# jenkinsm13/julia-spira

Measured on AMD Instinct MI355X. Metric: Msamples/sec at 1920x1080 spp=64 depth=8; fraction of HBM roofline, higher is better.
Workload: dtype f64

## Files before the change

### include/spira_hip.h

```cpp
#ifndef SPIRA_HIP_H
#define SPIRA_HIP_H

#include <stdint.h>

#ifdef __cplusplus
extern "C" {
#endif

#define SPIRA_ABI_VERSION 3

#define SPIRA_OK            0
#define SPIRA_E_INVALID    -1
#define SPIRA_E_NO_DEVICE  -2
#define SPIRA_E_HIP        -3
#define SPIRA_E_LIMIT      -4
#define SPIRA_E_UNSUPPORTED -5

#define SPIRA_SEM_MASK          0x0000000Fu
#define SPIRA_SEM_A             0x00000000u
#define SPIRA_SEM_CPU           0x00000001u
#define SPIRA_SEM_METAL         0x00000002u
#define SPIRA_SEM_HYBRID        0x00000003u
#define SPIRA_KERNEL_MASK       0x000000F0u
#define SPIRA_KERNEL_DEFAULT    0x00000000u
// ... 233 lines not shown
int spira_render_adaptive_f64(const double *spheres5, const double *materials8, const double *triangles10,
                              const double camera12[12], const spira_params *params, const spira_adaptive *adaptive,
                              double *out_hdr, double *out_img, uint32_t *out_spp, double *out_q);
int spira_render_adaptive_scene_f32(const spira_scene *scene, const float camera12[12], const spira_params *params, const spira_adaptive *adaptive,
                                    float *out_hdr, float *out_img, uint32_t *out_spp, float *out_q);
int spira_render_adaptive_scene_f64(const spira_scene *scene, const double camera12[12], const spira_params *params, const spira_adaptive *adaptive,
                                    double *out_hdr, double *out_img, uint32_t *out_spp, double *out_q);
int spira_render_adaptive_scene_device_f32(const spira_scene *scene, const float camera12[12], const spira_params *params, const spira_adaptive *adaptive,
                                           float *d_out_hdr, float *d_out_img, uint32_t *d_out_spp, float *d_out_q, void *stream);
int spira_render_adaptive_scene_device_f64(const spira_scene *scene, const double camera12[12], const spira_params *params, const spira_adaptive *adaptive,
                                           double *d_out_hdr, double *d_out_img, uint32_t *d_out_spp, double *d_out_q, void *stream);
int spira_adaptive_converged_f32(const float sum3[3], float q, uint32_t n, double tolerance, double floor);
int spira_adaptive_converged_f64(const double sum3[3], double q, uint32_t n, double tolerance, double floor);

int spira_sky_pixel_f64(const double camera12[12], uint32_t width, uint32_t height, uint32_t i, uint32_t j, const double *spheres5, uint32_t n_spheres);

int spira_render_features_f32(const float *spheres5, const float *materials8, const float *triangles10,
                              const float camera12[12], const spira_params *params,
                              float *out_albedo, float *out_normal, float *out_depth);
int spira_render_features_f64(const double *spheres5, const double *materials8, const double *triangles10,
                              const double camera12[12], const spira_params *params,
                              double *out_albedo, double *out_normal, double *out_depth);
int spira_render_features_scene_f32(const spira_scene *scene, const float camera12[12], const spira_params *params,
                                    float *out_albedo, float *out_normal, float *out_depth);
int spira_render_features_scene_f64(const spira_scene *scene, const double camera12[12], const spira_params *params,
                                    double *out_albedo, double *out_normal, double *out_depth);
int spira_render_features_scene_device_f32(const spira_scene *scene, const float camera12[12], const spira_params *params,
                                           float *d_out_albedo, float *d_out_normal, float *d_out_depth, void *stream);
int spira_render_features_scene_device_f64(const spira_scene *scene, const double camera12[12], const spira_params *params,
                                           double *d_out_albedo, double *d_out_normal, double *d_out_depth, void *stream);
// ... 30 lines not shown
```

### julia-spira_amd/csrc/spira_device.h

```cpp
#pragma once
#include <hip/hip_runtime.h>
#include <stdint.h>
#include <type_traits>
#include "spira_fastdiv.h"
#include "spira_sky.h"

namespace spira {

__device__ __forceinline__ float sqrt_rn(float x) { return __builtin_sqrtf(x); }
__device__ __forceinline__ double sqrt_rn(double x) { return __builtin_sqrt(x); }

constexpr int kBlock = 256;
#ifndef SPIRA_WAVES_F32
#define SPIRA_WAVES_F32 5
#endif
#ifndef SPIRA_WAVES_F64
#define SPIRA_WAVES_F64 4
#endif
#define SPIRA_WAVES_PER_SIMD(T) (sizeof(T) == 8 ? SPIRA_WAVES_F64 : SPIRA_WAVES_F32)
constexpr uint32_t kMaxTries = 64;

template <class T> struct Vec { T x, y, z; };

template <class T> __device__ __forceinline__ Vec<T> mk(T x, T y, T z) { Vec<T> r; r.x = x; r.y = y; r.z = z; return r; }
// ... 723 lines not shown
    if (TRI && sc.n_triangles) {
        Pack4<T> v0n = sc.tri[0], e1n = sc.tri[1], e2n = sc.tri[2];
#pragma unroll 2
        for (uint32_t i = 0; i < sc.n_triangles; ++i) {
            const Pack4<T> v0 = v0n, e1 = e1n, e2 = e2n;
            const uint32_t nx = i + 1 < sc.n_triangles ? i + 1 : i;
            v0n = sc.tri[3 * nx]; e1n = sc.tri[3 * nx + 1]; e2n = sc.tri[3 * nx + 2];
            T t;
            if (triangle_test<T>(v0, e1, e2, o, d, t_min, closest, t, pol)) {
                closest = t; prim = (int)(sc.n_spheres + i);
            }
        }
    }
}

template <class T>
__device__ __forceinline__ bool mesh_box_hit(const SceneLds<T> &sc, Vec<T> o, Vec<T> d, T closest) {
    const Vec<T> inv = mk<T>(rcp_fast(d.x), rcp_fast(d.y), rcp_fast(d.z));
    return box_entry<T>(sc.bvh_root[0], sc.bvh_root[1], o, inv, closest) >= (T)0;
}

template <class T>
__device__ __forceinline__ void closest_hit_local(const SceneLds<T> &sc, Vec<T> o, Vec<T> d, T t_min, T &closest, int &prim) {
    ExactDiv exact;
    closest_hit_local<T>(sc, o, d, t_min, closest, prim, exact);
}
template <class T, bool BVH, class P, bool TRI = true>
__device__ __forceinline__ int closest_hit(const SceneLds<T> &sc, Vec<T> o, Vec<T> d, T t_min, T &t_hit, uint32_t &slot, P &pol) {
    T closest; int prim;
    closest_hit_local<T, P, TRI>(sc, o, d, t_min, closest, prim, pol);
// ... 236 lines not shown
    uint32_t pl = q - slot * rc.tile_pixels;
    uint32_t lr = fastdiv(pl, rc.fd_width);
    uint32_t lx = pl - lr * rc.width;
    j = ref_row_j(rc, lr);
    i = lx + 1;
    pixel = (j - 1) * rc.width + lx;
    sample = rc.sample0 + pass * rc.slots + slot;
}

template <class T> struct RayQueue { Pack4<T> *A; Pack4<T> *B; Pack2<T> *C; };

struct Stats {
    unsigned long long segments, rays_enqueued, radiance_rmw, radiance_store, redone_waves, rays_parked;
    unsigned long long mesh_wave_trips, mesh_lane_trips;
    unsigned long long sky_pixels;
};

template <class T> struct BounceArgs {
    SceneGlobal<T> scene;
    RenderConst<T> rc;
    RayQueue<T> qin, qout;
    Pack3<T> *L;
    const uint32_t *cnt_in;
    uint32_t *cnt_out;
    uint32_t *blk_stats;
    uint32_t cap;
    Stats *stats;
    uint32_t bounce;
    uint32_t pass;
    uint32_t n_first;
// ... 257 lines not shown
    Pack4<T> *mesh_list;
    uint32_t mesh_min_batch;
    uint32_t refill_free;
    uint32_t mesh_mode;
    uint32_t *mesh_count;
    uint32_t resume_k, resume_nw;
    uint32_t *redo;
    uint32_t redo_only;
    Stats *stats;
    Pack4<T> *accum;
    FastDiv fd_keff;
    uint32_t k_eff;
    uint32_t accum_first;
    uint32_t l_private;
    uint32_t sky_runs;
};

#ifndef SPIRA_RESOLVE_RUN
#define SPIRA_RESOLVE_RUN 4
#endif
__device__ __forceinline__ uint32_t owned_pixel(uint32_t w, uint32_t nw, uint32_t l) {
    constexpr uint32_t kRun = SPIRA_RESOLVE_RUN;
    static_assert(64 % kRun == 0, "a run length divides the wave");
    return ((l / kRun) * nw + w) * kRun + l % kRun;
}

template <class T>
__device__ __forceinline__ void resolve_pixel(Pack4<T> *accum, const Pack3<T> *L, uint32_t tile_pixels, uint32_t k_eff, bool first_pass, uint32_t p) {
    Pack4<T> acc;
    if (first_pass) { acc.x = 0; acc.y = 0; acc.z = 0; acc.w = 0; } else acc = accum[p];
// ... 104 lines not shown
    const bool mixed = mesh_mode != 0u || rc.max_depth <= 128u;
    const uint32_t dense_pct = mixed ? a.dense_pct : 0u;
    const bool defer = mesh_mode != 0u || (BVH && mixed && a.mesh_list != nullptr);
    Pack4<T> *mlist = a.mesh_list + 3 * (size_t)region;
    uint32_t n_rmw = 0, n_store = 0, n_seg = 0, n_enq = 0, n_park = 0;
    uint32_t n_wtrips = 0, n_ltrips = 0;
    uint32_t n_in = 0;
    const bool own = !BVH && !EXT && !TRI && sizeof(T) == 8 && a.accum != nullptr;
    const uint32_t n_own = own ? 64u * a.k_eff : 0u;
    const uint32_t n_sub_first = own ? (n_own + SUB - 1) / SUB : (a.n_first + SUB - 1) / SUB;
    const bool priv = kCarry && own && a.l_private != 0;
    const uint32_t l_base = priv ? wid * n_own : 0u;
    constexpr bool kOwnT = !BVH && !EXT && !TRI && sizeof(T) == 8;
    uint32_t sky_mask = 0;
    uint32_t *sky_word = reinterpret_cast<uint32_t *>(cam_lds + 12) + wave;
    static_assert(12 * sizeof(T) + WPB * sizeof(uint32_t) <= 128 || !kOwnT, "a word per wave behind the camera");
    if constexpr (kOwnT) {
        if (own && a.sky_runs) {
            constexpr uint32_t kRun = SPIRA_RESOLVE_RUN, kRuns = 64 / kRun, kRowSlots = 64 / kRun;
            static_assert(kRun == 4 && 2 * 64 * sizeof(Pack3<T>) <= SUB * sizeof(Pack4<T>), "the run mask below is written for runs of 4; a row of terms fits the work list");
            {
                const uint32_t px = owned_pixel(wid, NW, lane);
                bool sky = false;
                if (px < rc.tile_pixels) {
                    uint32_t pi, pj, pixel, sample;
                    path_of<T>(rc, px, a.pass, pi, pj, pixel, sample);
                    sky = sky_pixel(cam_lds, rc.width, rc.height, pi, pj, a.scene.spheres5, a.scene.n_spheres);
                }
                unsigned long long b = __ballot(sky);
                b &= b >> 1; b &= b >> 2;
                for (uint32_t g = 0; g < kRuns; ++g) sky_mask |= (uint32_t)((b >> (kRun * g)) & 1ull) << g;
            }
            Pack3<T> *s_sky = reinterpret_cast<Pack3<T> *>(s_rnd);
            for (uint32_t m = sky_mask; m; m &= m - 1u) {
                const uint32_t g = (uint32_t)__builtin_ctz(m);
                const uint32_t px = owned_pixel(wid, NW, g * kRun + lane % kRun);
                uint32_t pi, pj, pixel, sample0;
                path_of<T>(rc, px, a.pass, pi, pj, pixel, sample0);
                Pack3<T> acc;
                acc.x = 0; acc.y = 0; acc.z = 0;
                if (!a.accum_first && lane < kRun) { const Pack4<T> a0 = a.accum[px]; acc.x = a0.x; acc.y = a0.y; acc.z = a0.z; }
                for (uint32_t s0 = 0; s0 < a.k_eff; s0 += kRowSlots) {
                    const uint32_t slot = s0 + lane / kRun;
                    if (slot < a.k_eff) {
                        Vec<T> o_, d_;
                        camera_ray_lds<T>(rc, cam_lds, pix_div, pi, pj, pixel, sample0 + slot, o_, d_, pol);
                        const Vec<T> c = sky_term_x<T, EXT>(d_, mk<T>(1, 1, 1), nullptr);
                        Pack3<T> l; l.x = c.x; l.y = c.y; l.z = c.z;
                        s_sky[lane] = l;
                        ++n_seg; ++n_store;
                    }
                    wave_lds_sync();
                    if (lane < kRun) {
                        const uint32_t n = a.k_eff - s0 < kRowSlots ? a.k_eff - s0 : kRowSlots;
                        for (uint32_t k = 0; k < n; ++k) { const Pack3<T> l = s_sky[k * kRun + lane]; acc.x = acc.x + l.x; acc.y = acc.y + l.y; acc.z = acc.z + l.z; }
                    }
                    wave_lds_sync();
                }
                if (lane < kRun) a.L[priv ? l_base + g * a.k_eff * kRun + lane : px] = acc;
            }
        }
        if (own) { if (lane == 0) *sky_word = sky_mask; wave_lds_sync(); }
    }

    auto park = [&](uint32_t slot_i, const Vec<T> o_, const Vec<T> d_, const Vec<T> beta_, T closest_, uint32_t q_, int prim_, uint32_t stage_hit) {
        Pack4<T> A, B, C;
        A.x = o_.x; A.y = o_.y; A.z = o_.z; A.w = d_.x;
        B.x = d_.y; B.y = d_.z; B.z = beta_.x; B.w = beta_.y;
        C.x = beta_.z; C.y = closest_; C.z = Bits<T>::from_u32(q_); C.w = Bits<T>::from_u32((uint32_t)(prim_ + 1) | (stage_hit << kStageShift));
        mlist[3 * (size_t)slot_i] = A; mlist[3 * (size_t)slot_i + 1] = B; mlist[3 * (size_t)slot_i + 2] = C;
    };
    uint32_t mfill = 0;
    constexpr int kMaxSeg = 16;
    uint32_t pfx[kMaxSeg + 1];
    bool segmented = false;
    {
        uint32_t cnt = 0;
// ... 26 lines not shown
            Vec<T> o[R], beta[R];
            Pending<T> pend[R];
            ExtState<T> ex[R];
            uint32_t q[R], ent[R], stg[R], ref[R];
            uint32_t ka[R], kb[R];
            bool valid[R];
#pragma unroll
            for (int r = 0; r < R; ++r) {
                const uint32_t idx = sub * SUB + r * 64 + lane;
                valid[r] = false; stg[r] = round; ref[r] = 0; q[r] = 0; ka[r] = 0; kb[r] = 0;
                pend[r].kind = kDead; pend[r].rough = 0; pend[r].v = mk<T>(0, 0, 0);
                o[r] = mk<T>(0, 0, 0); beta[r] = mk<T>(1, 1, 1);
                bool parked = false; T park_t = 0; int park_prim = -1;
                uint32_t qf = idx;
                bool in = idx < limit;
                if (own && first) {
                    const uint32_t t = idx / SPIRA_RESOLVE_RUN, run = fastdiv(t, a.fd_keff);
                    const uint32_t px = owned_pixel(wid, NW, run * SPIRA_RESOLVE_RUN + idx % SPIRA_RESOLVE_RUN);
                    qf = (t - run * a.k_eff) * rc.tile_pixels + px;
                    in = in && px < rc.tile_pixels;
                    if constexpr (kOwnT) in = in && !((*sky_word >> run) & 1u);
                }
                const uint32_t ql = priv ? l_base + idx : qf;
                if (in) {
                    if (first) {
                        uint32_t pixel, sample, pi, pj;
                        Vec<T> d;
                        q[r] = ql;
                        path_of<T>(rc, qf, a.pass, pi, pj, pixel, sample);
                        if (kCarry) { ka[r] = mix32(rc.sA + pixel) ^ (sample << 8); kb[r] = mix32(rc.sB ^ pixel) + (sample << 8); }
                        camera_ray_lds<T>(rc, cam_lds, pix_div, pi, pj, pixel, sample, o[r], d, pol);
                        if (EXT) { ex[r].flags = rc.flags; if (rc.flags & kExtSpectral) beta[r] = ext_wavelength<T>(sc, rc.sA, rc.sB, pixel, sample, ex[r]); }
                        T t; uint32_t slot = 0;
                        int prim;
                        if (defer) {
                            if (kCam && a.cam_consts) closest_hit_local<T, Pol, TRI, true>(sc, o[r], d, (T)0.001, t, prim, pol, cam_sph);
                            else closest_hit_local<T, Pol, TRI>(sc, o[r], d, (T)0.001, t, prim, pol);
                            parked = mesh_box_hit<T>(sc, o[r], d, t);
                        } else if (kCam && !BVH && a.cam_consts) { closest_hit_local<T, Pol, TRI, true>(sc, o[r], d, (T)0.001, t, prim, pol, cam_sph); }
                        else prim = closest_hit<T, BVH, Pol, TRI>(sc, o[r], d, (T)0.001, t, slot, pol);
                        ++n_seg;
                        if (parked) { park_t = t; park_prim = prim; pend[r].v = d; }
                        else if (prim < 0) {
                            const Vec<T> c = sky_term_x<T, EXT>(d, beta[r], &ex[r]);
                            Pack3<T> l; l.x = c.x; l.y = c.y; l.z = c.z;
                            a.L[ql] = l;
                            ++n_store;
                        } else {
                            valid[r] = true;
                            o[r] = o[r] + d * t;
                            ref[r] = (BVH && prim >= (int)ref_base) ? ref_base + slot : (uint32_t)prim;
                            pend[r].v = d;
                        }
                    } else {
// ... 364 lines not shown
        const uint32_t px = owned_pixel(wid, NW, lane);
        bool summed = false;
        if constexpr (kOwnT) sky_mask = (uint32_t)__builtin_amdgcn_readfirstlane((int)*sky_word);
        if constexpr (kOwnT) summed = ((sky_mask >> (lane / SPIRA_RESOLVE_RUN)) & 1u) != 0;
        if (summed) {
            const Pack3<T> l = a.L[priv ? l_base + (lane / SPIRA_RESOLVE_RUN) * a.k_eff * SPIRA_RESOLVE_RUN + lane % SPIRA_RESOLVE_RUN : px];
            Pack4<T> acc;
            if (a.accum_first) acc.w = 0; else acc = a.accum[px];
            acc.x = l.x; acc.y = l.y; acc.z = l.z;
            a.accum[px] = acc;
        } else if (px < rc.tile_pixels) {
            if (priv) resolve_pixel_run<T>(a.accum, a.L + l_base + (lane / SPIRA_RESOLVE_RUN) * a.k_eff * SPIRA_RESOLVE_RUN + lane % SPIRA_RESOLVE_RUN, a.k_eff, a.accum_first != 0, px);
            else resolve_pixel<T>(a.accum, a.L, rc.tile_pixels, a.k_eff, a.accum_first != 0, px);
        }
        const uint32_t seg = __shfl(n_seg, 0), rmw = __shfl(n_rmw, 0), sto = __shfl(n_store, 0);
        if (lane < 4) {
            unsigned long long *f = lane == 0 ? &a.stats->segments : (lane == 1 ? &a.stats->rays_enqueued : (lane == 2 ? &a.stats->radiance_rmw : &a.stats->radiance_store));
            atomicAdd(f, (unsigned long long)(lane == 0 ? seg : (lane == 1 ? n_enq : (lane == 2 ? rmw : sto))));
        }
        if constexpr (kOwnT) if (lane == 4 && sky_mask) atomicAdd(&a.stats->sky_pixels, (unsigned long long)(SPIRA_RESOLVE_RUN * __popc(sky_mask)));
    }
    MESH_STAT(if (lane == 0) { unsigned long long *g = g_mesh_dbg + (mesh_mode == 2u ? 16 : 0);
                               atomicAdd(&g[0], __builtin_readcyclecounter() - dbg_t0); atomicAdd(&g[1], dbg_sess); atomicAdd(&g[2], (unsigned long long)dbg_ns);
                               atomicAdd(&g[3], (unsigned long long)dbg_ws); atomicAdd(&g[4], (unsigned long long)dbg_ls); atomicAdd(&g[5], (unsigned long long)dbg_rf);
                               atomicAdd(&g[6], (unsigned long long)dbg_rays); atomicAdd(&g[7], (unsigned long long)dbg_rounds); atomicAdd(&g[9], dbg_walk); atomicAdd(&g[10], 1ull); atomicAdd(&g[11], (unsigned long long)dbg_ws1); atomicAdd(&g[12], (unsigned long long)dbg_ls1);
                               atomicAdd(&g[8], (unsigned long long)dbg_h[0]); atomicAdd(&g[13], (unsigned long long)dbg_h[1]); atomicAdd(&g[14], (unsigned long long)dbg_h[2]); atomicAdd(&g[15], (unsigned long long)dbg_h[3]); })
    if (lane == 0) {
        if (mesh_mode == 2u) {
            const uint32_t row = 4 * wid * kseg;
            a.blk_stats[row] += n_seg; a.blk_stats[row + 1] += n_rmw; a.blk_stats[row + 2] += n_store; a.blk_stats[row + 3] += n_enq;
        } else {
            a.blk_stats[4 * wid] = n_seg;
            a.blk_stats[4 * wid + 1] = n_rmw;
            a.blk_stats[4 * wid + 2] = n_store;
            a.blk_stats[4 * wid + 3] = n_enq;
// ... 824 lines not shown
```

### julia-spira_amd/csrc/spira_hip.hip

```cpp
#include <hip/hip_runtime.h>
#include <sys/mman.h>
#include <rccl/rccl.h>
#include <dlfcn.h>

#include <algorithm>
#include <atomic>
#include <chrono>
#include <cmath>
#include <cstdio>
#include <cstdlib>
#include <cstring>
#include <condition_variable>
#include <mutex>
#include <new>
#include <string>
#include <thread>
#include <type_traits>
#include <vector>

#include "../../include/spira_hip.h"
#include "../../include/spira_spd.h"
#include "spira_device.h"
#include "spira_bvh.h"
#include "spira_validate.h"
// ... 132 lines not shown
    struct LbvhSmall *h_lbvh = nullptr;
    std::vector<void *> lbvh_retired;
    SceneStore scene;
    spira::Stats *h_stats = nullptr;
    void *h_stage = nullptr; size_t h_stage_cap = 0;
    std::vector<hipEvent_t> stage_ev;
    hipEvent_t ev_start = nullptr, ev_stop = nullptr;
    hipEvent_t ev_done = nullptr;
    bool have_done = false;
    std::vector<hipEvent_t> ev_pool;
    size_t ev_used = 0;
    std::vector<hipEvent_t> ev_mid;
    std::vector<size_t> ev_mid_end;
    size_t ev_mid_used = 0;
    spira_counters last{};
    uint64_t last_sky_pixels = 0;
    bool last_valid = false, last_pending = false;
    hipStream_t last_stream = nullptr;
    std::recursive_mutex mu;
};

constexpr int kMaxDevices = 16;
inline Ctx g_ctx[kMaxDevices];

}
using namespace spira_host;
namespace spira_tu {
int lbvh_topology(Ctx &c, hipStream_t st, uint32_t n, const LbvhWs &w, LbvhTopo &out);
}

// ... 478 lines not shown

spira::Knobs read_knobs() {
    spira::Knobs k;
    k.batch_rays = env_u32("SPIRA_BATCH_RAYS", k.batch_rays);
    k.R = env_u32("SPIRA_R", k.R);
    k.blocks_per_cu = env_u32("SPIRA_BLOCKS_PER_CU", 0);
    k.defer_mesh = env_u32("SPIRA_DEFER_MESH", 1); k.mesh_two_pass = env_u32("SPIRA_MESH_TWO_PASS", 1);
    k.fused_resolve = env_u32("SPIRA_FUSED_RESOLVE", 1); k.private_l = env_u32("SPIRA_PRIVATE_L", 1);
    k.spec_div = env_u32("SPIRA_SPEC_DIV", 1);
    k.dense_pct = std::min<uint32_t>(env_u32("SPIRA_DENSE_PCT", 70), 100);
    k.mesh_min_batch = std::max<uint32_t>(1, env_u32("SPIRA_MESH_MIN_BATCH", 128));
    k.mesh_refill = std::min<uint32_t>(64, std::max<uint32_t>(1, env_u32("SPIRA_MESH_REFILL", 16)));
    k.mesh_fat_waves_per_cu = env_u32("SPIRA_MESH_FAT_WAVES_PER_CU", 16);
    k.cam_consts = env_u32("SPIRA_CAM_CONSTS", 1);
    k.sky_runs = env_u32("SPIRA_SKY_RUNS", 1);
    return k;
}
template <class T>
spira::PlanIn plan_input(const Ctx &c, const spira_params *p, uint32_t rows, uint32_t nt_scene, bool progressive, bool caller_rng, bool out_on_device) {
    spira::PlanIn in;
    in.width = p->width; in.rows = rows; in.spp = p->spp; in.max_depth = p->max_depth; in.flags = p->flags; in.batch_rays = p->batch_rays;
    in.n_triangles = nt_scene; in.num_cus = (uint32_t)c.num_cus;
    in.progressive = progressive; in.caller_rng = caller_rng; in.out_on_device = out_on_device;
    in.prec = sizeof(T); in.block = spira::kBlock; in.waves_per_simd = SPIRA_WAVES_PER_SIMD(T); in.carry_key = SPIRA_CARRY_KEY;
    in.pack4 = sizeof(spira::Pack4<T>); in.pack3 = sizeof(spira::Pack3<T>); in.pack2 = sizeof(spira::Pack2<T>);
    in.k = read_knobs();
    return in;
}

int ensure_workspaces(Ctx &c, const spira::Workspace &w) {
// ... 191 lines not shown
    *stat_rows = G * plan.wpb;
    for (int i = 0; i < 2; ++i) {
        pa.q[i] = k.queue(i);
        pa.qref[i] = (uint32_t *)c.qR[i].p;
        pa.qkey[i] = (uint2 *)c.qK[i].p;
    }
    pa.blk_stats = (uint32_t *)c.blkstats.p;
    pa.stats = k.stats();
    if (k.spec) pa.redo = k.redo();
    pa.mesh_mode = 0; pa.mesh_count = nullptr; pa.resume_k = 1; pa.resume_nw = 0;
    pa.mesh_min_batch = kn.mesh_min_batch;
    pa.refill_free = kn.mesh_refill;
    size_t lds_a = k.lds + (size_t)plan.wpb * plan.sub * sizeof(P4) + 128;
    pa.cam_consts = (kn.cam_consts && pa.scene.n_spheres && lds_a + (size_t)pa.scene.n_spheres * sizeof(P4) <= (size_t)160 * 1024) ? 1u : 0u;
    if (pa.cam_consts) lds_a += (size_t)pa.scene.n_spheres * sizeof(P4);
    if (plan.two_pass) {
        pa.mesh_mode = 1; pa.mesh_count = (uint32_t *)c.mesh_count.p;
        pa.resume_nw = G * plan.wpb; pa.resume_k = plan.fat_k(pa.resume_nw);
    }
    if (plan.fused) {
        pa.accum = k.accum(); pa.k_eff = plan.k_eff(pa.pass); pa.fd_keff = spira::fastdiv_make(pa.k_eff);
        pa.accum_first = (pa.pass == 0 && !k.progressive) ? 1u : 0u;
        pa.l_private = plan.l_private ? 1u : 0u;
        pa.sky_runs = plan.sky_runs ? 1u : 0u;
    }
    if (int rc = verify_path_args<T>(c, pa, G)) return rc;
    HIP_TRY(hipEventRecord(c.ev_pool[c.ev_used++], k.st));
    if (int rc = launch_path<T>((int)plan.R, dim3(G), lds_a, k.st, pa, k.spec)) return rc;
    k.launches += k.spec ? 2 : 1;
    if (pa.mesh_mode == 1) {
// ... 1949 lines not shown
    if (c.last_pending) {
        HIP_TRY(hipEventSynchronize(c.ev_stop));
        HIP_TRY(hipStreamSynchronize(c.last_stream));
        float ms = 0;
        HIP_TRY(hipEventElapsedTime(&ms, c.ev_start, c.ev_stop));
        c.last.kernel_ms = ms;
        c.last.segments = c.h_stats->segments;
        c.last.rays_enqueued = c.h_stats->rays_enqueued;
        c.last.radiance_rmw = c.h_stats->radiance_rmw;
        c.last.radiance_stores = c.h_stats->radiance_store;
        c.last.redone_waves = c.h_stats->redone_waves;
        c.last.rays_parked = c.h_stats->rays_parked;
        c.last.mesh_wave_trips = c.h_stats->mesh_wave_trips;
        c.last.mesh_lane_trips = c.h_stats->mesh_lane_trips;
        c.last_sky_pixels = c.h_stats->sky_pixels;
        double wms = 0;
        for (size_t i = 0; i < c.ev_mid_used; ++i) {
            float m = 0;
            HIP_TRY(hipEventElapsedTime(&m, c.ev_mid[i], c.ev_pool[c.ev_mid_end[i]]));
            wms += m;
        }
        c.last.walk_kernel_ms = wms;
        double bms = 0;
        for (size_t i = 0; i + 1 < c.ev_used; i += 2) {
            float m = 0;
            HIP_TRY(hipEventElapsedTime(&m, c.ev_pool[i], c.ev_pool[i + 1]));
            bms += m;
        }
        c.last.bounce_kernel_ms = bms;
        c.last_pending = false;
    }
    *out = c.last;
    return 0;
}

int spira_get_sky_pixels(uint64_t *out) {
    if (!out) return fail(SPIRA_E_INVALID, "out is NULL");
    spira_counters unused;
    if (int rc = spira_get_counters(&unused)) return rc;
    Ctx *cp = nullptr;
    if (int rc = get_ctx(&cp)) return rc;
    std::lock_guard<std::recursive_mutex> lock(cp->mu);
    *out = cp->last_sky_pixels;
    return 0;
}

void spira_shutdown(void) {
    { std::lock_guard<std::mutex> rl(g_rccl.mu); if (g_rccl.handle) rccl_release(g_rccl); }
    for (int d = 0; d < kMaxDevices; ++d) {
        Ctx &c = g_ctx[d];
        std::lock_guard<std::recursive_mutex> lock(c.mu);
        if (!c.init) continue;
        (void)hipSetDevice(d);
        (void)hipDeviceSynchronize();
        for (int i = 0; i < 2; ++i) { c.qA[i].release(); c.qB[i].release(); c.qC[i].release(); c.qR[i].release(); c.qK[i].release(); c.qX[i].release(); }
        c.mesh_list.release(); c.mesh_count.release();
        c.redo.release(); c.L.release(); c.accum.release(); c.counts.release(); c.blkstats.release(); c.stats.release(); c.scene.release(); c.out_tmp.release(); c.trace.release(); c.rng.release(); c.multi_tile.release(); c.multi_stack.release(); c.multi_full.release(); c.spd32.release(); c.spd64.release(); c.hyb_state.release(); c.hyb_mat.release(); c.hyb_flags.release();
        c.ad_q.release(); c.ad_n.release(); c.ad_list[0].release(); c.ad_list[1].release(); c.ad_count.release();
// ... 164 lines not shown
}
int spira_render_adaptive_scene_device_f32(const spira_scene *scene, const float cam[12], const spira_params *p, const spira_adaptive *adaptive,
                                           float *d_hdr, float *d_img, uint32_t *d_spp, float *d_q, void *stream) {
    if (!scene) return fail(SPIRA_E_INVALID, "scene handle is NULL or was destroyed");
    return render_adaptive_entry<float>(scene, nullptr, nullptr, nullptr, cam, p, adaptive, d_hdr, d_img, d_spp, d_q, true, stream);
}
int spira_render_adaptive_scene_device_f64(const spira_scene *scene, const double cam[12], const spira_params *p, const spira_adaptive *adaptive,
                                           double *d_hdr, double *d_img, uint32_t *d_spp, double *d_q, void *stream) {
    if (!scene) return fail(SPIRA_E_INVALID, "scene handle is NULL or was destroyed");
    return render_adaptive_entry<double>(scene, nullptr, nullptr, nullptr, cam, p, adaptive, d_hdr, d_img, d_spp, d_q, true, stream);
}
int spira_sky_pixel_f64(const double cam[12], uint32_t width, uint32_t height, uint32_t i, uint32_t j, const double *spheres5, uint32_t n_spheres) {
    if (!cam || (n_spheres && !spheres5)) return fail(SPIRA_E_INVALID, "cam or spheres5 is NULL");
    return spira::sky_pixel(cam, width, height, i, j, spheres5, n_spheres) ? 1 : 0;
}
int spira_adaptive_converged_f32(const float sum3[3], float q, uint32_t n, double tolerance, double floor) {
    return adaptive_converged_host<float>(sum3, q, n, tolerance, floor);
}
int spira_adaptive_converged_f64(const double sum3[3], double q, uint32_t n, double tolerance, double floor) {
    return adaptive_converged_host<double>(sum3, q, n, tolerance, floor);
}

int spira_render_features_f32(const float *s, const float *m, const float *t, const float cam[12], const spira_params *p,
                              float *out_albedo, float *out_normal, float *out_depth) {
    return features_entry<float>(nullptr, s, m, t, cam, p, out_albedo, out_normal, out_depth, false, nullptr);
}
int spira_render_features_f64(const double *s, const double *m, const double *t, const double cam[12], const spira_params *p,
                              double *out_albedo, double *out_normal, double *out_depth) {
    return features_entry<double>(nullptr, s, m, t, cam, p, out_albedo, out_normal, out_depth, false, nullptr);
}
// ... 73 lines not shown
```

### julia-spira_amd/csrc/spira_plan.h

```cpp
#pragma once
#include <algorithm>
#include <cstdint>

#include "../../include/spira_hip.h"

namespace spira {

struct Knobs {
    uint32_t batch_rays = 160u << 20;
    uint32_t R = 2;
    uint32_t blocks_per_cu = 0;
    uint32_t defer_mesh = 1, mesh_two_pass = 1, fused_resolve = 1, private_l = 1;
    uint32_t spec_div = 1;
    uint32_t dense_pct = 70, mesh_min_batch = 128, mesh_refill = 16, mesh_fat_waves_per_cu = 16, cam_consts = 1;
    uint32_t sky_runs = 1;
};

struct PlanIn {
    uint32_t width = 0, rows = 0;
    uint32_t spp = 0, max_depth = 0, flags = 0, batch_rays = 0;
    uint32_t n_triangles = 0;
    uint32_t num_cus = 0;
    bool progressive = false, caller_rng = false, out_on_device = false;
    bool adaptive = false;
    uint32_t prec = 0, block = 0, waves_per_simd = 0, carry_key = 0;
    uint32_t pack4 = 0, pack3 = 0, pack2 = 0;
    Knobs k;
};

enum class Org { Black, Hybrid, MetalWavefront, Metal, Cpu, Mega, Path, Bounce };
// ... 3 lines not shown
struct Workspace {
    uint64_t queue4 = 0, queue2 = 0, q_ref = 0, q_key = 0, q_x = 0;
    uint64_t mesh_list = 0, mesh_count = 0, redo = 0, blkstats = 0, L = 0, counts = 0, accum = 0, out_tmp = 0, rng = 0;
    uint64_t hyb_state = 0, hyb_mat = 0, hyb_flags = 0;
};

struct Plan {
    PlanIn in;
    Org org = Org::Black;
    uint32_t R = 2, wpb = 0, sub = 0, max_blocks = 0;
    uint64_t tile_pixels = 0, batch = 0;
    uint32_t slots = 0, n_pass = 0;
    bool mesh_scene = false, defer_mesh = false, two_pass = false;
    bool fused = false, l_private = false;
    bool sky_runs = false;
    bool spec_allowed = false;
    uint32_t G_max = 0, cap_max = 0;
    uint64_t q_rays = 0;
    uint32_t ppw = 0, G_metal = 0;
    Workspace ws;

    Geometry geometry(uint64_t n_first) const {
        if (fused) {
            const uint64_t k = n_first / tile_pixels;
            return {(uint32_t)((tile_pixels + 64 * wpb - 1) / (64 * wpb)), (uint32_t)((64 * k + sub - 1) / sub * sub)};
        }
        const uint64_t n_sub = (n_first + sub - 1) / sub;
        const uint32_t G = (uint32_t)std::min<uint64_t>((n_sub + wpb - 1) / wpb, max_blocks);
        const uint64_t nw = (uint64_t)G * wpb;
        return {G, (uint32_t)(((n_sub + nw - 1) / nw) * sub)};
// ... 41 lines not shown
    pl.R = (k.R == 1 && !ext) ? 1 : 2;
    pl.mesh_scene = in.n_triangles > SPIRA_LDS_TRIANGLES;
    pl.defer_mesh = persistent && pl.mesh_scene && in.max_depth <= 128 && k.defer_mesh != 0;
    pl.two_pass = pl.defer_mesh && k.mesh_two_pass != 0;

    const uint32_t blocks_per_cu = k.blocks_per_cu ? k.blocks_per_cu : !persistent ? 16 : (pl.mesh_scene && !pl.two_pass) ? 4 : 32;
    pl.max_blocks = (uint32_t)std::min<uint64_t>((uint64_t)in.num_cus * blocks_per_cu, 0x7FFFFFFFull);
    pl.wpb = in.block / 64;
    pl.sub = 64 * pl.R;
    pl.fused = persistent && in.prec == 8 && pl.R == 2 && in.n_triangles == 0 && !ext && pl.slots <= 64 && k.fused_resolve != 0 && !in.adaptive;
    const Geometry g = pl.geometry(pl.batch);
    pl.G_max = g.G; pl.cap_max = g.cap;
    const uint64_t waves = (uint64_t)g.G * pl.wpb;
    pl.l_private = pl.fused && in.carry_key && in.max_depth <= 128 && k.private_l != 0 && 64ull * waves * pl.slots <= 0x7FFFFFFFull;
    pl.sky_runs = pl.fused && k.sky_runs != 0;
    pl.q_rays = (uint64_t)g.cap * waves;
    if (pl.q_rays > 0xFFFFFFFFull) return bad("pass too large");
    pl.spec_allowed = pl.org == Org::Cpu || (pl.org == Org::Metal && !in.progressive) || (pl.org == Org::MetalWavefront && !in.progressive && pl.R == 2) ||
                      (persistent && pl.R == 2);
    if (in.max_depth == 0) pl.org = Org::Black;

    Workspace &w = pl.ws;
    const uint64_t redo_per_wave = (pl.spec_allowed && k.spec_div) ? sizeof(uint32_t) : 0, stat_row = 4 * sizeof(uint32_t);
    w.accum = tp * in.pack4;
    w.out_tmp = in.out_on_device ? 0 : 2 * 3 * tp * in.prec;
    if (in.caller_rng && !in.out_on_device) w.rng = tp * sizeof(uint32_t);
    switch (pl.org) {
    case Org::Black: break;
    case Org::Hybrid:
        if (tp > 0xFFFFFFFFull / 2) return bad("image too large for SPIRA_SEM_HYBRID");
// ... 345 lines not shown
```

### julia-spira_amd/csrc/spira_sky.h

```cpp
#pragma once
#include <stdint.h>
#include "spira_fastdiv.h"

namespace spira {

SPIRA_HD inline bool sky_pixel(const double *cam, uint32_t W, uint32_t H, uint32_t i, uint32_t j, const double *spheres5, uint32_t n_spheres) {
    const double kSlack = 1.0 / 1048576.0, kHuge = 1.0e100, kTiny = 1.0e-100;
    const double w1 = (double)W - 1.0, h1 = (double)H - 1.0;
    const double uc = ((double)i - 0.5) / w1, vc = ((double)j - 0.5) / h1;
    const double hn = __builtin_sqrt((cam[6] * cam[6] + cam[7] * cam[7]) + cam[8] * cam[8]);
    const double vn = __builtin_sqrt((cam[9] * cam[9] + cam[10] * cam[10]) + cam[11] * cam[11]);
    const double rho = (0.5 * (hn / w1 + vn / h1)) * (1.0 + kSlack);
    const double dx = ((cam[3] + cam[6] * uc) + cam[9] * vc) - cam[0];
    const double dy = ((cam[4] + cam[7] * uc) + cam[10] * vc) - cam[1];
    const double dz = ((cam[5] + cam[8] * uc) + cam[11] * vc) - cam[2];
    const double dd = (dx * dx + dy * dy) + dz * dz, dn = __builtin_sqrt(dd);
    if (!(rho >= 0.0 && dn > rho && dn > kTiny && dn < kHuge)) return false;
    const double q = __builtin_sqrt(dd - rho * rho);
    for (uint32_t s = 0; s < n_spheres; ++s) {
        const double *sp = spheres5 + 5 * (uint64_t)s;
        const double r = sp[3];
        const double cx = sp[0] - cam[0], cy = sp[1] - cam[1], cz = sp[2] - cam[2];
        const double cn = __builtin_sqrt((cx * cx + cy * cy) + cz * cz);
        const double xx = cy * dz - cz * dy, xy = cz * dx - cx * dz, xz = cx * dy - cy * dx;
        const double xn = __builtin_sqrt((xx * xx + xy * xy) + xz * xz);
        const double cd = __builtin_fabs((cx * dx + cy * dy) + cz * dz);
        if (!(r > 0.0 && r < kHuge && cn > kTiny && cn < kHuge)) return false;
        if (!(xn * q - cd * rho > (r * (1.0 + kSlack) + cn * kSlack) * dd)) return false;
    }
    return true;
}

}
```

### julia-spira_amd/spira_hip/_binding.py

```python
import ctypes as C
import os
import subprocess

import numpy as np

_HERE = os.path.dirname(os.path.abspath(__file__))
CSRC = os.path.normpath(os.path.join(_HERE, "..", "csrc"))
LIB_PATH = os.environ.get("SPIRA_HIP_LIB", os.path.join(CSRC, "libspira_hip.so"))

ABI_VERSION = 3

SEM_A, SEM_CPU, SEM_METAL, SEM_HYBRID = 0x0, 0x1, 0x2, 0x3
KERNEL_DEFAULT, KERNEL_MEGA, KERNEL_BOUNCE, KERNEL_WAVEFRONT = 0x00, 0x10, 0x20, 0x30
POST_ACES, POST_ACES_GAMMA, POST_CLAMP_GAMMA, POST_NONE = 0x000, 0x100, 0x200, 0x300
ROWS_BOTTOM_UP = 0x1000
FLAG_PROFILE = 0x10000
EXT_DIELECTRIC, EXT_SPECTRAL = 0x20000, 0x40000
MAX_RAYS = 1 << 26
RAY_MISS, RAY_INVALID = -1, -3
CAST_INPLACE = 0x1
MAX_HITS = 16
HITS_COUNT_ALL = 0x2
CAM_PINHOLE, CAM_THIN_LENS, CAM_ORTHO = 0, 1, 2
MAX_DEPTH, MAX_SPP = 255, 1 << 24

EXPORTS = [
    "spira_abi_version", "spira_build_id", "spira_last_error", "spira_device_count", "spira_set_device", "spira_get_counters",
    "spira_get_sky_pixels", "spira_sky_pixel_f64",
    "spira_shutdown", "spira_camera_lookat_f32", "spira_camera_lookat_f64", "spira_render_f32", "spira_render_f64",
    "spira_render_device_f32", "spira_render_device_f64", "spira_trace_paths_f32", "spira_trace_paths_f64",
    "spira_tonemap_f32", "spira_stripe_rows", "spira_accumulate_f32", "spira_accumulate_f64", "spira_accumulate_device_f32",
    "spira_accumulate_device_f64", "spira_scene_create_f32", "spira_scene_create_f64", "spira_scene_destroy",
    "spira_render_scene_f32", "spira_render_scene_f64", "spira_render_scene_device_f32", "spira_render_scene_device_f64",
    "spira_render_multi_f32", "spira_render_multi_f64", "spira_scene_create_multi_f32", "spira_scene_create_multi_f64",
    "spira_render_multi_scene_f32", "spira_render_multi_scene_f64",
    "spira_render_adaptive_f32", "spira_render_adaptive_f64", "spira_render_adaptive_scene_f32", "spira_render_adaptive_scene_f64",
    "spira_render_adaptive_scene_device_f32", "spira_render_adaptive_scene_device_f64", "spira_adaptive_converged_f32", "spira_adaptive_converged_f64",
    "spira_render_features_f32", "spira_render_features_f64", "spira_render_features_scene_f32", "spira_render_features_scene_f64",
    "spira_render_features_scene_device_f32", "spira_render_features_scene_device_f64",
    "spira_denoise_f32", "spira_denoise_f64", "spira_denoise_device_f32", "spira_denoise_device_f64",
    "spira_scene_update_f32", "spira_scene_update_f64", "spira_scene_update_device_f32", "spira_scene_update_device_f64",
    "spira_scene_rebuild_f32", "spira_scene_rebuild_f64", "spira_scene_rebuild_device_f32", "spira_scene_rebuild_device_f64",
    "spira_scene_cast_f32", "spira_scene_cast_f64", "spira_scene_cast_device_f32", "spira_scene_cast_device_f64",
# ... 133 lines not shown
    return d


def sky_pixel(camera12, width, height, i, j, spheres5):
    cam = np.ascontiguousarray(camera12, dtype=np.float64)
    sp = np.ascontiguousarray(spheres5, dtype=np.float64).reshape(-1, 5)
    assert cam.shape == (12,)
    fn = lib().spira_sky_pixel_f64
    fn.argtypes = [C.c_void_p, C.c_uint32, C.c_uint32, C.c_uint32, C.c_uint32, C.c_void_p, C.c_uint32]
    rc = fn(cam.ctypes.data_as(C.c_void_p), width, height, i, j, sp.ctypes.data_as(C.c_void_p), len(sp))
    if rc < 0:
        _check(rc)
    return rc


def stripe_rows(height, stripe_h, stripe_count, stripe_rank):
    return lib().spira_stripe_rows(height, stripe_h, stripe_count, stripe_rank)


def camera_lookat(position, look_at, up, fov_deg, aspect_ratio, focus_dist=1.0, prec="f32"):
    npdt, cdt = _dt(prec)
    p, pp = _arr(position, npdt)
    l, lp = _arr(look_at, npdt)
    u, up_ = _arr(up, npdt)
    out = np.zeros(12, dtype=npdt)
    if prec == "f32":
        _check(lib().spira_camera_lookat_f32(pp, lp, up_, cdt(fov_deg), cdt(aspect_ratio), out.ctypes.data_as(C.c_void_p)))
    else:
        _check(lib().spira_camera_lookat_f64(pp, lp, up_, cdt(fov_deg), cdt(aspect_ratio), cdt(focus_dist),
                                             out.ctypes.data_as(C.c_void_p)))
# ... 522 lines not shown
```

Measured before the change: 28900.

## Cull camera-ray sphere tests with per-pixel conservative sphere reach masks

Extends the per-pixel sky test so it returns a bitmask of spheres each pixel's camera cone could reach. In the fused f64 path the masks are OR-combined over runs of four pixels and stored in LDS. First-bounce camera rays then test only spheres in their wave's combined mask. This cuts redundant ray-sphere intersection work on primary rays, at the cost of extra LDS, a mask computation per owned pixel, shuffles, and a new stats counter.

```diff
diff --git a/include/spira_hip.h b/include/spira_hip.h
--- a/include/spira_hip.h
+++ b/include/spira_hip.h
@@ -271,6 +271,9 @@
 int spira_adaptive_converged_f64(const double sum3[3], double q, uint32_t n, double tolerance, double floor);
 
 int spira_sky_pixel_f64(const double camera12[12], uint32_t width, uint32_t height, uint32_t i, uint32_t j, const double *spheres5, uint32_t n_spheres);
+int spira_sphere_mask_pixel_f64(const double camera12[12], uint32_t width, uint32_t height, uint32_t i, uint32_t j, const double *spheres5, uint32_t n_spheres,
+                                uint32_t *out_mask);
+int spira_get_cam_tests_skipped(uint64_t *out);
 
 int spira_render_features_f32(const float *spheres5, const float *materials8, const float *triangles10,
                               const float camera12[12], const spira_params *params,
diff --git a/julia-spira_amd/csrc/spira_device.h b/julia-spira_amd/csrc/spira_device.h
--- a/julia-spira_amd/csrc/spira_device.h
+++ b/julia-spira_amd/csrc/spira_device.h
@@ -761,6 +761,45 @@
     }
 }
 
+template <class T, class P>
+__device__ __forceinline__ void closest_hit_cam_masked(const SceneLds<T> &sc, Vec<T> d, T t_min, T &closest, int &prim, P &pol, const Pack4<T> *cam, uint32_t mask) {
+    closest = (T)INFINITY;
+    prim = -1;
+    const T a = dot(d, d);
+    const T two_a = (T)2.0 * a;
+    const T four_a = (T)4 * a;
+    const RootDiv<T> over_2a = root_divisor<T>(two_a, pol);
+    root_t_min<T>(t_min, pol);
+    const uint32_t n = sc.n_spheres;
+    uint32_t m = mask;
+    uint32_t s = m ? (uint32_t)__builtin_ctz(m) : n;
+    Pack4<T> c_next = cam[s < n ? s : 0u];
+#pragma unroll 2
+    while (s < n) {
+        const Pack4<T> c = c_next;
+        m &= m - 1u;
+        const uint32_t sn = m ? (uint32_t)__builtin_ctz(m) : n;
+        c_next = cam[sn < n ? sn : s];
+        const Vec<T> oc = mk<T>(c.x, c.y, c.z);
+        const T cc = c.w;
+        T b = (T)2.0 * dot(oc, d);
+        const T bb = b * b;
+        T disc = bb - four_a * cc;
+        if (!(disc < 0)) {
+            root_operands<T>(bb, disc, pol);
+            T sq = root_sqrt<T>(disc, pol);
+            T root = root_over<T>(-b - sq, over_2a, pol);
+            bool ok = !(root < t_min || root > closest);
+            if (!ok && root < t_min) {
+                root = root_over<T>(-b + sq, over_2a, pol);
+                ok = !(root < t_min || root > closest);
+            }
+            if (ok) { closest = root; prim = (int)s; }
+        }
+        s = sn;
+    }
+}
+
 template <class T>
 __device__ __forceinline__ bool mesh_box_hit(const SceneLds<T> &sc, Vec<T> o, Vec<T> d, T closest) {
     const Vec<T> inv = mk<T>(rcp_fast(d.x), rcp_fast(d.y), rcp_fast(d.z));
@@ -1027,6 +1066,7 @@
     unsigned long long segments, rays_enqueued, radiance_rmw, radiance_store, redone_waves, rays_parked;
     unsigned long long mesh_wave_trips, mesh_lane_trips;
     unsigned long long sky_pixels;
+    unsigned long long cam_tests_skipped;
 };
 
 template <class T> struct BounceArgs {
@@ -1314,6 +1354,7 @@
     uint32_t accum_first;
     uint32_t l_private;
     uint32_t sky_runs;
+    uint32_t cam_cull;
 };
 
 #ifndef SPIRA_RESOLVE_RUN
@@ -1448,22 +1489,29 @@
     constexpr bool kOwnT = !BVH && !EXT && !TRI && sizeof(T) == 8;
     uint32_t sky_mask = 0;
     uint32_t *sky_word = reinterpret_cast<uint32_t *>(cam_lds + 12) + wave;
-    static_assert(12 * sizeof(T) + WPB * sizeof(uint32_t) <= 128 || !kOwnT, "a word per wave behind the camera");
+    static_assert(12 * sizeof(T) + 2 * WPB * sizeof(uint32_t) <= 128 || !kOwnT, "two words per wave behind the camera");
+    uint32_t *run_words = reinterpret_cast<uint32_t *>(cam_sph + a.scene.n_spheres) + wave * (64 / SPIRA_RESOLVE_RUN);
     if constexpr (kOwnT) {
-        if (own && a.sky_runs) {
+        uint32_t run_mask = a.scene.n_spheres >= 32u ? 0xFFFFFFFFu : (1u << a.scene.n_spheres) - 1u;
+        if (own && (a.sky_runs || a.cam_cull == 1u)) {
             constexpr uint32_t kRun = SPIRA_RESOLVE_RUN, kRuns = 64 / kRun, kRowSlots = 64 / kRun;
-            static_assert(kRun == 4 && 2 * 64 * sizeof(Pack3<T>) <= SUB * sizeof(Pack4<T>), "the run mask below is written for runs of 4; a row of terms fits the work list");
+            static_assert(kRun == 4 && 2 * 64 * sizeof(Pack3<T>) <= SUB * sizeof(Pack4<T>), "the run masks below are written for runs of 4; a row of terms fits the work list");
             {
                 const uint32_t px = owned_pixel(wid, NW, lane);
                 bool sky = false;
+                uint32_t pm = 0;
                 if (px < rc.tile_pixels) {
                     uint32_t pi, pj, pixel, sample;
                     path_of<T>(rc, px, a.pass, pi, pj, pixel, sample);
-                    sky = sky_pixel(cam_lds, rc.width, rc.height, pi, pj, a.scene.spheres5, a.scene.n_spheres);
+                    sky = !pixel_may_reach(cam_lds, rc.width, rc.height, pi, pj, a.scene.spheres5, a.scene.n_spheres, pm);
+                    pm &= run_mask;
                 }
-                unsigned long long b = __ballot(sky);
-                b &= b >> 1; b &= b >> 2;
-                for (uint32_t g = 0; g < kRuns; ++g) sky_mask |= (uint32_t)((b >> (kRun * g)) & 1ull) << g;
+                if (a.cam_cull == 1u) { pm |= (uint32_t)__shfl_xor((int)pm, 1); pm |= (uint32_t)__shfl_xor((int)pm, 2); run_mask = pm; }
+                if (a.sky_runs) {
+                    unsigned long long b = __ballot(sky);
+                    b &= b >> 1; b &= b >> 2;
+                    for (uint32_t g = 0; g < kRuns; ++g) sky_mask |= (uint32_t)((b >> (kRun * g)) & 1ull) << g;
+                }
             }
             Pack3<T> *s_sky = reinterpret_cast<Pack3<T> *>(s_rnd);
             for (uint32_t m = sky_mask; m; m &= m - 1u) {
@@ -1494,7 +1542,13 @@
                 if (lane < kRun) a.L[priv ? l_base + g * a.k_eff * kRun + lane : px] = acc;
             }
         }
-        if (own) { if (lane == 0) *sky_word = sky_mask; wave_lds_sync(); }
+        uint32_t skipped = 0;
+        if (own && a.cam_cull) {
+            if (lane % SPIRA_RESOLVE_RUN == 0) run_words[lane / SPIRA_RESOLVE_RUN] = run_mask;
+            if (owned_pixel(wid, NW, lane) < rc.tile_pixels && !((sky_mask >> (lane / SPIRA_RESOLVE_RUN)) & 1u)) skipped = a.k_eff * (a.scene.n_spheres - (uint32_t)__popc(run_mask));
+            for (int sft = 32; sft > 0; sft >>= 1) skipped += __shfl_down(skipped, sft);
+        }
+        if (own) { if (lane == 0) { *sky_word = sky_mask; sky_word[WPB] = skipped; } wave_lds_sync(); }
     }
 
     auto park = [&](uint32_t slot_i, const Vec<T> o_, const Vec<T> d_, const Vec<T> beta_, T closest_, uint32_t q_, int prim_, uint32_t stage_hit) {
@@ -1551,6 +1605,14 @@
                 bool parked = false; T park_t = 0; int park_prim = -1;
                 uint32_t qf = idx;
                 bool in = idx < limit;
+                uint32_t cam_mask = 0xFFFFFFFFu;
+                if constexpr (kOwnT) if (own && first && a.cam_cull) {
+                    const uint32_t e0 = sub * SUB + (uint32_t)r * 64u;
+                    const uint32_t g0 = fastdiv(e0 / SPIRA_RESOLVE_RUN, a.fd_keff), g1 = fastdiv((e0 + 63u) / SPIRA_RESOLVE_RUN, a.fd_keff);
+                    uint32_t mm = 0;
+                    for (uint32_t g = g0; g <= g1 && g < 64u / SPIRA_RESOLVE_RUN; ++g) mm |= run_words[g];
+                    cam_mask = (uint32_t)__builtin_amdgcn_readfirstlane((int)mm);
+                }
                 if (own && first) {
                     const uint32_t t = idx / SPIRA_RESOLVE_RUN, run = fastdiv(t, a.fd_keff);
                     const uint32_t px = owned_pixel(wid, NW, run * SPIRA_RESOLVE_RUN + idx % SPIRA_RESOLVE_RUN);
@@ -1574,7 +1636,12 @@
                             if (kCam && a.cam_consts) closest_hit_local<T, Pol, TRI, true>(sc, o[r], d, (T)0.001, t, prim, pol, cam_sph);
                             else closest_hit_local<T, Pol, TRI>(sc, o[r], d, (T)0.001, t, prim, pol);
                             parked = mesh_box_hit<T>(sc, o[r], d, t);
-                        } else if (kCam && !BVH && a.cam_consts) { closest_hit_local<T, Pol, TRI, true>(sc, o[r], d, (T)0.001, t, prim, pol, cam_sph); }
+                        } else if (kCam && !BVH && a.cam_consts) {
+                            bool masked = false;
+                            if constexpr (kOwnT) masked = own && a.cam_cull != 0u;
+                            if (masked) closest_hit_cam_masked<T, Pol>(sc, d, (T)0.001, t, prim, pol, cam_sph, cam_mask);
+                            else closest_hit_local<T, Pol, TRI, true>(sc, o[r], d, (T)0.001, t, prim, pol, cam_sph);
+                        }
                         else prim = closest_hit<T, BVH, Pol, TRI>(sc, o[r], d, (T)0.001, t, slot, pol);
                         ++n_seg;
                         if (parked) { park_t = t; park_prim = prim; pend[r].v = d; }
@@ -1969,11 +2036,17 @@
             else resolve_pixel<T>(a.accum, a.L, rc.tile_pixels, a.k_eff, a.accum_first != 0, px);
         }
         const uint32_t seg = __shfl(n_seg, 0), rmw = __shfl(n_rmw, 0), sto = __shfl(n_store, 0);
-        if (lane < 4) {
+        if constexpr (kOwnT) {
+            const uint32_t skp = sky_word[WPB];
+            if (lane < 6) {
+                unsigned long long *f = lane == 0 ? &a.stats->segments : (lane == 1 ? &a.stats->rays_enqueued : (lane == 2 ? &a.stats->radiance_rmw : (lane == 3 ? &a.stats->radiance_store :
+                                        (lane == 4 ? &a.stats->sky_pixels : &a.stats->cam_tests_skipped))));
+                atomicAdd(f, (unsigned long long)(lane == 0 ? seg : (lane == 1 ? n_enq : (lane == 2 ? rmw : (lane == 3 ? sto : (lane == 4 ? (uint32_t)(SPIRA_RESOLVE_RUN * __popc(sky_mask)) : skp))))));
+            }
+        } else if (lane < 4) {
             unsigned long long *f = lane == 0 ? &a.stats->segments : (lane == 1 ? &a.stats->rays_enqueued : (lane == 2 ? &a.stats->radiance_rmw : &a.stats->radiance_store));
             atomicAdd(f, (unsigned long long)(lane == 0 ? seg : (lane == 1 ? n_enq : (lane == 2 ? rmw : sto))));
         }
-        if constexpr (kOwnT) if (lane == 4 && sky_mask) atomicAdd(&a.stats->sky_pixels, (unsigned long long)(SPIRA_RESOLVE_RUN * __popc(sky_mask)));
     }
     MESH_STAT(if (lane == 0) { unsigned long long *g = g_mesh_dbg + (mesh_mode == 2u ? 16 : 0);
                                atomicAdd(&g[0], __builtin_readcyclecounter() - dbg_t0); atomicAdd(&g[1], dbg_sess); atomicAdd(&g[2], (unsigned long long)dbg_ns);
diff --git a/julia-spira_amd/csrc/spira_hip.hip b/julia-spira_amd/csrc/spira_hip.hip
--- a/julia-spira_amd/csrc/spira_hip.hip
+++ b/julia-spira_amd/csrc/spira_hip.hip
@@ -170,6 +170,7 @@
     std::vector<size_t> ev_mid_end;
     size_t ev_mid_used = 0;
     spira_counters last{};
+    uint64_t last_cam_tests_skipped = 0;
     uint64_t last_sky_pixels = 0;
     bool last_valid = false, last_pending = false;
     hipStream_t last_stream = nullptr;
@@ -678,6 +679,7 @@
     k.mesh_fat_waves_per_cu = env_u32("SPIRA_MESH_FAT_WAVES_PER_CU", 16);
     k.cam_consts = env_u32("SPIRA_CAM_CONSTS", 1);
     k.sky_runs = env_u32("SPIRA_SKY_RUNS", 1);
+    k.cam_cull = env_u32("SPIRA_CAM_CULL", 1);
     return k;
 }
 template <class T>
@@ -899,6 +901,10 @@
     size_t lds_a = k.lds + (size_t)plan.wpb * plan.sub * sizeof(P4) + 128;
     pa.cam_consts = (kn.cam_consts && pa.scene.n_spheres && lds_a + (size_t)pa.scene.n_spheres * sizeof(P4) <= (size_t)160 * 1024) ? 1u : 0u;
     if (pa.cam_consts) lds_a += (size_t)pa.scene.n_spheres * sizeof(P4);
+    if (plan.fused && pa.cam_consts && pa.scene.n_spheres <= 32 && lds_a + (size_t)plan.wpb * 64 <= (size_t)160 * 1024) {
+        pa.cam_cull = plan.cam_cull ? 1u : 2u;
+        lds_a += (size_t)plan.wpb * 64;
+    }
     if (plan.two_pass) {
         pa.mesh_mode = 1; pa.mesh_count = (uint32_t *)c.mesh_count.p;
         pa.resume_nw = G * plan.wpb; pa.resume_k = plan.fat_k(pa.resume_nw);
@@ -2878,6 +2884,7 @@
         c.last.mesh_wave_trips = c.h_stats->mesh_wave_trips;
         c.last.mesh_lane_trips = c.h_stats->mesh_lane_trips;
         c.last_sky_pixels = c.h_stats->sky_pixels;
+        c.last_cam_tests_skipped = c.h_stats->cam_tests_skipped;
         double wms = 0;
         for (size_t i = 0; i < c.ev_mid_used; ++i) {
             float m = 0;
@@ -2906,6 +2913,17 @@
     if (int rc = get_ctx(&cp)) return rc;
     std::lock_guard<std::recursive_mutex> lock(cp->mu);
     *out = cp->last_sky_pixels;
+    return 0;
+}
+
+int spira_get_cam_tests_skipped(uint64_t *out) {
+    if (!out) return fail(SPIRA_E_INVALID, "out is NULL");
+    spira_counters unused;
+    if (int rc = spira_get_counters(&unused)) return rc;
+    Ctx *cp = nullptr;
+    if (int rc = get_ctx(&cp)) return rc;
+    std::lock_guard<std::recursive_mutex> lock(cp->mu);
+    *out = cp->last_cam_tests_skipped;
     return 0;
 }
 
@@ -3100,6 +3118,12 @@
     if (!cam || (n_spheres && !spheres5)) return fail(SPIRA_E_INVALID, "cam or spheres5 is NULL");
     return spira::sky_pixel(cam, width, height, i, j, spheres5, n_spheres) ? 1 : 0;
 }
+int spira_sphere_mask_pixel_f64(const double cam[12], uint32_t width, uint32_t height, uint32_t i, uint32_t j, const double *spheres5, uint32_t n_spheres,
+                                uint32_t *out_mask) {
+    if (!cam || !out_mask || (n_spheres && !spheres5)) return fail(SPIRA_E_INVALID, "cam, spheres5 or out_mask is NULL");
+    *out_mask = spira::sphere_mask_pixel(cam, width, height, i, j, spheres5, n_spheres);
+    return 0;
+}
 int spira_adaptive_converged_f32(const float sum3[3], float q, uint32_t n, double tolerance, double floor) {
     return adaptive_converged_host<float>(sum3, q, n, tolerance, floor);
 }
diff --git a/julia-spira_amd/csrc/spira_plan.h b/julia-spira_amd/csrc/spira_plan.h
--- a/julia-spira_amd/csrc/spira_plan.h
+++ b/julia-spira_amd/csrc/spira_plan.h
@@ -14,6 +14,7 @@
     uint32_t spec_div = 1;
     uint32_t dense_pct = 70, mesh_min_batch = 128, mesh_refill = 16, mesh_fat_waves_per_cu = 16, cam_consts = 1;
     uint32_t sky_runs = 1;
+    uint32_t cam_cull = 1;
 };
 
 struct PlanIn {
@@ -47,6 +48,7 @@
     bool mesh_scene = false, defer_mesh = false, two_pass = false;
     bool fused = false, l_private = false;
     bool sky_runs = false;
+    bool cam_cull = false;
     bool spec_allowed = false;
     uint32_t G_max = 0, cap_max = 0;
     uint64_t q_rays = 0;
@@ -118,6 +120,7 @@
     const uint64_t waves = (uint64_t)g.G * pl.wpb;
     pl.l_private = pl.fused && in.carry_key && in.max_depth <= 128 && k.private_l != 0 && 64ull * waves * pl.slots <= 0x7FFFFFFFull;
     pl.sky_runs = pl.fused && k.sky_runs != 0;
+    pl.cam_cull = pl.fused && k.cam_consts != 0 && k.cam_cull != 0;
     pl.q_rays = (uint64_t)g.cap * waves;
     if (pl.q_rays > 0xFFFFFFFFull) return bad("pass too large");
     pl.spec_allowed = pl.org == Org::Cpu || (pl.org == Org::Metal && !in.progressive) || (pl.org == Org::MetalWavefront && !in.progressive && pl.R == 2) ||
diff --git a/julia-spira_amd/csrc/spira_sky.h b/julia-spira_amd/csrc/spira_sky.h
--- a/julia-spira_amd/csrc/spira_sky.h
+++ b/julia-spira_amd/csrc/spira_sky.h
@@ -4,8 +4,9 @@
 
 namespace spira {
 
-SPIRA_HD inline bool sky_pixel(const double *cam, uint32_t W, uint32_t H, uint32_t i, uint32_t j, const double *spheres5, uint32_t n_spheres) {
+SPIRA_HD inline bool pixel_may_reach(const double *cam, uint32_t W, uint32_t H, uint32_t i, uint32_t j, const double *spheres5, uint32_t n_spheres, uint32_t &mask) {
     const double kSlack = 1.0 / 1048576.0, kHuge = 1.0e100, kTiny = 1.0e-100;
+    mask = 0xFFFFFFFFu;
     const double w1 = (double)W - 1.0, h1 = (double)H - 1.0;
     const double uc = ((double)i - 0.5) / w1, vc = ((double)j - 0.5) / h1;
     const double hn = __builtin_sqrt((cam[6] * cam[6] + cam[7] * cam[7]) + cam[8] * cam[8]);
@@ -15,8 +16,10 @@
     const double dy = ((cam[4] + cam[7] * uc) + cam[10] * vc) - cam[1];
     const double dz = ((cam[5] + cam[8] * uc) + cam[11] * vc) - cam[2];
     const double dd = (dx * dx + dy * dy) + dz * dz, dn = __builtin_sqrt(dd);
-    if (!(rho >= 0.0 && dn > rho && dn > kTiny && dn < kHuge)) return false;
+    if (!(rho >= 0.0 && dn > rho && dn > kTiny && dn < kHuge)) return true;
     const double q = __builtin_sqrt(dd - rho * rho);
+    bool any = false;
+    uint32_t m = 0;
     for (uint32_t s = 0; s < n_spheres; ++s) {
         const double *sp = spheres5 + 5 * (uint64_t)s;
         const double r = sp[3];
@@ -25,10 +28,22 @@
         const double xx = cy * dz - cz * dy, xy = cz * dx - cx * dz, xz = cx * dy - cy * dx;
         const double xn = __builtin_sqrt((xx * xx + xy * xy) + xz * xz);
         const double cd = __builtin_fabs((cx * dx + cy * dy) + cz * dz);
-        if (!(r > 0.0 && r < kHuge && cn > kTiny && cn < kHuge)) return false;
-        if (!(xn * q - cd * rho > (r * (1.0 + kSlack) + cn * kSlack) * dd)) return false;
+        const bool miss = (r > 0.0 && r < kHuge && cn > kTiny && cn < kHuge) && (xn * q - cd * rho > (r * (1.0 + kSlack) + cn * kSlack) * dd);
+        if (!miss) { any = true; m |= 1u << (s & 31u); }
     }
-    return true;
+    mask = m;
+    return any;
+}
+
+SPIRA_HD inline bool sky_pixel(const double *cam, uint32_t W, uint32_t H, uint32_t i, uint32_t j, const double *spheres5, uint32_t n_spheres) {
+    uint32_t mask;
+    return !pixel_may_reach(cam, W, H, i, j, spheres5, n_spheres, mask);
+}
+
+SPIRA_HD inline uint32_t sphere_mask_pixel(const double *cam, uint32_t W, uint32_t H, uint32_t i, uint32_t j, const double *spheres5, uint32_t n_spheres) {
+    uint32_t mask;
+    (void)pixel_may_reach(cam, W, H, i, j, spheres5, n_spheres, mask);
+    return n_spheres > 32u ? 0xFFFFFFFFu : mask;
 }
 
 }
diff --git a/julia-spira_amd/spira_hip/_binding.py b/julia-spira_amd/spira_hip/_binding.py
--- a/julia-spira_amd/spira_hip/_binding.py
+++ b/julia-spira_amd/spira_hip/_binding.py
@@ -26,7 +26,7 @@
 
 EXPORTS = [
     "spira_abi_version", "spira_build_id", "spira_last_error", "spira_device_count", "spira_set_device", "spira_get_counters",
-    "spira_get_sky_pixels", "spira_sky_pixel_f64",
+    "spira_get_sky_pixels", "spira_sky_pixel_f64", "spira_get_cam_tests_skipped", "spira_sphere_mask_pixel_f64",
     "spira_shutdown", "spira_camera_lookat_f32", "spira_camera_lookat_f64", "spira_render_f32", "spira_render_f64",
     "spira_render_device_f32", "spira_render_device_f64", "spira_trace_paths_f32", "spira_trace_paths_f64",
     "spira_tonemap_f32", "spira_stripe_rows", "spira_accumulate_f32", "spira_accumulate_f64", "spira_accumulate_device_f32",
@@ -190,6 +190,23 @@
     return rc
 
 
+def sphere_mask_pixel(camera12, width, height, i, j, spheres5):
+    cam = np.ascontiguousarray(camera12, dtype=np.float64)
+    sp = np.ascontiguousarray(spheres5, dtype=np.float64).reshape(-1, 5)
+    assert cam.shape == (12,)
+    fn = lib().spira_sphere_mask_pixel_f64
+    fn.argtypes = [C.c_void_p, C.c_uint32, C.c_uint32, C.c_uint32, C.c_uint32, C.c_void_p, C.c_uint32, C.c_void_p]
+    mask = C.c_uint32(0)
+    _check(fn(cam.ctypes.data_as(C.c_void_p), width, height, i, j, sp.ctypes.data_as(C.c_void_p), len(sp), C.byref(mask)))
+    return mask.value
+
+
+def cam_tests_skipped():
+    n = C.c_uint64(0)
+    _check(lib().spira_get_cam_tests_skipped(C.byref(n)))
+    return n.value
+
+
 def stripe_rows(height, stripe_h, stripe_count, stripe_rank):
     return lib().spira_stripe_rows(height, stripe_h, stripe_count, stripe_rank)
 
```

After: 29150, median of 6. Within noise of the previous version (+0.9%).
